# url-kaist/Quatro

Measured on NVIDIA H100. Metric: registrations/sec (64-ring pair), higher is better.
Workload: dtype f32 (front end, match, graph filter) / f64 (graph boundary, GNC, COTE)

## Files before the change

quatro_b200/csrc/api.cu:

```cuda
#include <cmath>
#include <new>
#include <stddef.h>
#include <stdio.h>
#include <stdlib.h>
#include <string.h>
#include <algorithm>
#include <map>
#include <mutex>
#include <utility>
#include <vector>

#include "handle.cuh"

using namespace qb;

namespace {

__global__ void wave_init_kernel(int* ctr_block, int n_ints, int* bbox, int n_clouds) {
  const int i = blockIdx.x * blockDim.x + threadIdx.x;
  if (i < n_ints) ctr_block[i] = 0;
  if (i < n_clouds * 6) bbox[i] = (i % 6) < 3 ? INT_MAX : INT_MIN;
}

__global__ void cache_copy_kernel(int to_cache, const int* __restrict__ slot_of_cloud, int V, float4* __restrict__ w_vox, float4* __restrict__ w_nrm,
// ... 75 lines not shown
  QB_CUDA_TRY(L, L->val_a.alloc(n_sort > n_hist ? n_sort : n_hist));
  QB_CUDA_TRY(L, L->val_b.alloc(n_sort));
  QB_CUDA_TRY(L, L->aos_scratch.alloc(2 * V * kDescDim));
  L->cub_bytes = sort_temp_bytes((int)(C * V));
  QB_CUDA_TRY(L, L->cub_temp.alloc_bytes(L->cub_bytes));
  QB_CUDA_TRY(L, L->vox_start.alloc(C * (V + 1)));
  QB_CUDA_TRY(L, L->vox_pts.alloc(C * V));
  QB_CUDA_TRY(L, L->cell_key.alloc(C * V));
  QB_CUDA_TRY(L, L->cell_start.alloc(C * (V + 1)));
  QB_CUDA_TRY(L, L->normals.alloc(C * V));
  QB_CUDA_TRY(L, L->spfh.alloc(C * V * kDescPad));
  QB_CUDA_TRY(L, L->nbr_list.alloc(C * kNbrGlobalCap * V));
  QB_CUDA_TRY(L, L->nbr_cnt.alloc(C * V));
  QB_CUDA_TRY(L, L->desc_t.alloc(C * kDescK * V));
  QB_CUDA_TRY(L, cudaMemset(L->desc_t, 0, C * kDescK * V * sizeof(float)));
  QB_CUDA_TRY(L, L->desc_tiles.alloc(C * kDescK * V * 3));
  QB_CUDA_TRY(L, cudaMemset(L->desc_tiles, 0, C * kDescK * V * 3 * sizeof(float)));
  QB_CUDA_TRY(L, L->desc_norm.alloc(C * V));
  QB_CUDA_TRY(L, L->tc_fallback.alloc(S));
  QB_CUDA_TRY(L, L->tc_stats.alloc(32));
  QB_CUDA_TRY(L, cudaMemset(L->tc_stats, 0, 32 * sizeof(unsigned long long)));
  QB_CUDA_TRY(L, L->rowbest.alloc(S * V));
  QB_CUDA_TRY(L, L->colpart.alloc(L->colpart_count()));
  QB_CUDA_TRY(L, L->colbest.alloc(S * V));
  QB_CUDA_TRY(L, L->mut_i.alloc(S * V));
  QB_CUDA_TRY(L, L->mut_j.alloc(S * V));
  QB_CUDA_TRY(L, L->mark.alloc(S * V));
  QB_CUDA_TRY(L, L->partner.alloc(S * V));
  QB_CUDA_TRY(L, L->mean.alloc(C * 4));
  QB_CUDA_TRY(L, L->corr_src.alloc(S * Lc));
  QB_CUDA_TRY(L, L->corr_tgt.alloc(S * Lc));
  QB_CUDA_TRY(L, L->ma.alloc(S * Lc));
// ... 1199 lines not shown
```

quatro_b200/csrc/common.cuh:

```cuda
#pragma once
#include <cuda_runtime.h>
#include <stdint.h>
#include <stdio.h>

#include "quatro_b200.h"

namespace qb {

constexpr int kOffIJ = 1 << 17;
constexpr int kOffK = 1 << 15;
constexpr uint64_t kCellMask = (1ull << 52) - 1;
constexpr uint64_t kCellInvalid = kCellMask;
constexpr int kCloudShift = 52;

__host__ __device__ __forceinline__ bool cell_ok(int i, int j, int k) {
  return i >= -kOffIJ && i < kOffIJ - 1 && j >= -kOffIJ && j < kOffIJ - 1 && k >= -kOffK && k < kOffK - 1;
}
__host__ __device__ __forceinline__ uint64_t cell_key(int i, int j, int k) {
  return ((uint64_t)(k + kOffK) << 36) | ((uint64_t)(j + kOffIJ) << 18) | (uint64_t)(i + kOffIJ);
}

constexpr int kVoxShift = 31;
constexpr uint64_t kVoxMask = (1ull << kVoxShift) - 1;
constexpr uint64_t kVoxInvalid = kVoxMask;
constexpr int kVsChunks = 64;
constexpr int kVsTile = 2048;

__device__ __forceinline__ bool raw_point_kept(const float4 p, int skip_flagged) {
  return isfinite(p.x) && isfinite(p.y) && isfinite(p.z) && !(skip_flagged && p.w < 0.0f);
}
__host__ __device__ __forceinline__ int vox_chunk_size(int n) { return n > 0 ? (n + kVsChunks - 1) / kVsChunks : 1; }

constexpr int kDescDim = 33;
constexpr int kDescPad = 36;
constexpr int kDescK = 40;
constexpr int kMatchTile = 128;
constexpr int kNbrGlobalCap = 80;

struct WaveCounters {
  int* n_valid;
  int* n_vox;
  int* n_lat;
  int* n_cells;
  int* cloud_status;
  int* bbox;
  int* vox_digits;
  int* n_mutual;
  int* n_corr;
  int* swapped;
  int* n_clique;
// ... 99 lines not shown
```

quatro_b200/csrc/tc_match.cu:

```cuda
#include "handle.cuh"
#include <cstdlib>

namespace qb {

constexpr int kTcM = 128, kTcN = 64;
constexpr int kTcBlk = 64;
constexpr int kTcKB = kDescK / 8;
constexpr int kTcTileBytes = kDescK * kTcBlk * 4;
constexpr int kTileFloats = kDescK * kTcBlk;
constexpr int kTcImages = 3;
constexpr int kTcEpiWarps = 8;
constexpr int kTcThreads = (kTcEpiWarps + 2) * 32;
constexpr int kTcDone = 4;
constexpr int kTcStages = 2;
constexpr int kTcSmemTiles = 256;
constexpr float kTcC = 1.2e-4f;
constexpr float kTcNormMax = 0x1p124f;
constexpr float kTcNormRel = 4.0e-6f;
constexpr int kSpinLimit = 400000;

__device__ __forceinline__ uint32_t smem_u32(const void* p) { return (uint32_t)__cvta_generic_to_shared(p); }

__device__ __forceinline__ uint64_t tc_smem_desc(uint32_t addr) {
  return (uint64_t)((addr & 0x3FFFF) >> 4) | ((uint64_t)((kTcBlk * 16) >> 4) << 16) | ((uint64_t)(128 >> 4) << 32);
}

__device__ __forceinline__ void wgmma_tf32_64x64x8(float (&d)[32], uint64_t adesc, uint64_t bdesc, int accumulate) {
  asm volatile(
      "{\n\t"
      ".reg .pred p;\n\t"
      "setp.ne.b32 p, %34, 0;\n\t"
      "wgmma.mma_async.sync.aligned.m64n64k8.f32.tf32.tf32 "
      "{%0, %1, %2, %3, %4, %5, %6, %7, %8, %9, %10, %11, %12, %13, %14, %15, "
      "%16, %17, %18, %19, %20, %21, %22, %23, %24, %25, %26, %27, %28, %29, %30, %31}, %32, %33, p, 1, 1;\n\t"
      "}\n"
      : "+f"(d[0]), "+f"(d[1]), "+f"(d[2]), "+f"(d[3]), "+f"(d[4]), "+f"(d[5]), "+f"(d[6]), "+f"(d[7]), "+f"(d[8]), "+f"(d[9]),
        "+f"(d[10]), "+f"(d[11]), "+f"(d[12]), "+f"(d[13]), "+f"(d[14]), "+f"(d[15]), "+f"(d[16]), "+f"(d[17]), "+f"(d[18]),
        "+f"(d[19]), "+f"(d[20]), "+f"(d[21]), "+f"(d[22]), "+f"(d[23]), "+f"(d[24]), "+f"(d[25]), "+f"(d[26]), "+f"(d[27]),
        "+f"(d[28]), "+f"(d[29]), "+f"(d[30]), "+f"(d[31])
      : "l"(adesc), "l"(bdesc), "r"(accumulate)
      : "memory");
}

__device__ __forceinline__ bool wg_all(bool v, int g) {
  uint32_t r;
  asm volatile(
      "{\n\t.reg .pred p, q;\n\t"
      "setp.ne.u32 p, %1, 0;\n\t"
      "bar.red.and.pred q, %2, 128, p;\n\t"
// ... 14 lines not shown
  uint32_t bits = 0xFFFFFFFFu;
  if (q < n_vox[cloud]) {
    const size_t base = (size_t)cloud * kDescK * V + q;
    float acc = 0.0f;
#pragma unroll
    for (int d = 0; d < kDescDim; ++d) {
      const float xc = desc_t[base + (size_t)d * V] - tc_mu(d);
      acc = __fmaf_rn(xc, xc, acc);
    }
    bits = acc == acc ? __float_as_uint(acc) : 0xFFFFFFFEu;
  }
  keys[(size_t)cloud * V + q] = ((uint64_t)cloud << 32) | bits;
  vals[(size_t)cloud * V + q] = (uint32_t)q;
}

__global__ void __launch_bounds__(256) split_desc_kernel(const float* __restrict__ desc_t, const int* __restrict__ n_vox, int V,
                                                         const uint32_t* __restrict__ perm, float* __restrict__ tiles,
                                                         float* __restrict__ norm, int* __restrict__ fallback) {
  const int cloud = blockIdx.y;
  const int q = blockIdx.x * blockDim.x + threadIdx.x;
  const int n = n_vox[cloud];
  const int NB = V / kTcBlk;
  if (q >= ((n + kTcM - 1) & ~(kTcM - 1))) return;
  const size_t base = (size_t)cloud * kDescK * V + (q < n ? perm[(size_t)cloud * V + q] : 0u);
  const int blk = q / kTcBlk, p = q % kTcBlk;
  float4* __restrict__ img = reinterpret_cast<float4*>(tiles + (size_t)(cloud * NB + blk) * kTcImages * kTileFloats) + p;
  const bool is_col = (cloud & 1) != 0;
  const float kLow = 1.0f - 0.5f * kTcC;
  float acc = 0.0f;
#pragma unroll
  for (int kc = 0; kc < kDescK / 4; ++kc) {
    float xv[4], hv[4], lv[4];
#pragma unroll
    for (int e = 0; e < 4; ++e) {
      const int d = 4 * kc + e;
      const bool live = d < kDescDim && q < n;
      const float x = live ? desc_t[base + (size_t)d * V] : 0.0f;
      const float xc = live ? x - tc_mu(d) : 0.0f;
      xv[e] = x;
      acc = __fmaf_rn(xc, xc, acc);
      float xs = is_col ? -2.0f * xc : xc;
      if (q < n && d == kDescDim) xs = is_col ? 1.0f : kLow * acc;
      if (q < n && d == kDescDim + 1) xs = is_col ? kLow * acc : 1.0f;
      hv[e] = __uint_as_float(__float_as_uint(xs) & 0xFFFFE000u);
      lv[e] = __uint_as_float(__float_as_uint(xs - hv[e]) & 0xFFFFE000u);
    }
    img[0 * (kTileFloats / 4) + kc * kTcBlk] = make_float4(hv[0], hv[1], hv[2], hv[3]);
    img[1 * (kTileFloats / 4) + kc * kTcBlk] = make_float4(lv[0], lv[1], lv[2], lv[3]);
    if (kc < kDescK / 4 - 1) img[2 * (kTileFloats / 4) + kc * kTcBlk] = make_float4(xv[0], xv[1], xv[2], xv[3]);
  }
  img[2 * (kTileFloats / 4) + (kDescK / 4 - 1) * kTcBlk] = make_float4(q < n ? kLow * acc : INFINITY, 0.0f, 0.0f, 0.0f);
  if (q < n) norm[(size_t)cloud * V + q] = acc;
  if (q < n && !(acc <= kTcNormMax)) fallback[cloud >> 1] = 1;
}

__global__ void __launch_bounds__(1024) dedup_kernel(const float* __restrict__ desc_t, const int* __restrict__ n_vox, int V,
                                                     const uint64_t* __restrict__ sorted_keys, const uint32_t* __restrict__ perm, int enable,
                                                     uint32_t* __restrict__ uperm, uint32_t* __restrict__ class_of, int* __restrict__ n_unique) {
  __shared__ int scan_smem[33];
  const int cloud = blockIdx.x;
  const int n = n_vox[cloud];
  const float* __restrict__ D = desc_t + (size_t)cloud * kDescK * V;
  const uint32_t* __restrict__ pm = perm + (size_t)cloud * V;
  const uint64_t* __restrict__ sk = sorted_keys + (size_t)cloud * V;
  int base = 0;
  for (int start = 0; start < n; start += blockDim.x) {
// ... 77 lines not shown
}
__device__ __forceinline__ unsigned tc_fkey(float f) {
  unsigned key = __float_as_uint(f);
  key = (key & 0x80000000u) ? ~key : (key | 0x80000000u);
  return f == f ? key : 0xFFFFFFFFu;
}
__device__ __forceinline__ float tc_fkey_inv(unsigned key) { return __uint_as_float((key & 0x80000000u) ? (key & 0x7FFFFFFFu) : ~key); }

template <bool kDbg, bool kProf = false>
__global__ void __launch_bounds__(kTcThreads, 2)
tc_nn_kernel(const float* __restrict__ tiles, const float* __restrict__ norm, const int* __restrict__ n_vox, int V,
             const uint32_t* __restrict__ perm, unsigned long long* __restrict__ rowbest, unsigned long long* __restrict__ colbest_r,
             unsigned* __restrict__ tile_cmax, int* __restrict__ fallback, unsigned long long* __restrict__ stats,
             float* __restrict__ dbg_tile) {
  extern __shared__ __align__(128) unsigned char smem[];
  __shared__ uint64_t s_fullx[kTcStages], s_sfree[kTcStages], s_fullhl, s_mma[kTcDone], s_afull;
  __shared__ unsigned long long s_rbest[kTcM];
  __shared__ __align__(16) float s_wcj[kTcEpiWarps][kTcN];
  __shared__ unsigned short s_queue[kTcEpiWarps][32];
  __shared__ int s_seq[8];
  __shared__ float s_tlb[kTcSmemTiles];
  __shared__ int s_dead, s_abort, s_evals, s_warm, s_npos;
  __shared__ int s_ndec;

  const int pair = blockIdx.y, stripe = blockIdx.x;
  const int cloudA = 2 * pair, cloudB = 2 * pair + 1;
  const int nA = n_vox[cloudA], nB = n_vox[cloudB];
  const int r0 = stripe * kTcM;
  if (r0 >= nA || nB <= 0) return;

  const int warp = threadIdx.x >> 5, lane = threadIdx.x & 31;
  const int NB = V / kTcBlk;
  auto tick = [&]() -> long long { return kProf ? clock64() : 0ll; };
  auto prof = [&](int slot, long long cyc) { if (kProf && lane == 0) atomicAdd(stats + slot, (unsigned long long)cyc); };
  const long long t_begin = tick();
  constexpr uint32_t kABytes = (kTcM / kTcBlk) * kTcImages * kTcTileBytes;
  constexpr uint32_t kHLBytes = 2 * kTcTileBytes;
  constexpr uint32_t kXBytes = kTcTileBytes;
  const uint32_t sA = smem_u32(smem), sHL = sA + kABytes, sX0 = sHL + kHLBytes;
  const float* __restrict__ tA = tiles + (size_t)cloudA * NB * kTcImages * kTileFloats;
  const float* __restrict__ tB = tiles + (size_t)cloudB * NB * kTcImages * kTileFloats;
  const float* __restrict__ nrmA = norm + (size_t)cloudA * V;
  const float* __restrict__ nrmB = norm + (size_t)cloudB * V;
  const uint32_t* __restrict__ permA = perm + (size_t)cloudA * V;
  const uint32_t* __restrict__ permB = perm + (size_t)cloudB * V;
  unsigned long long* __restrict__ cbg = colbest_r + (size_t)pair * V;
  const uint32_t bar_fullx0 = smem_u32(&s_fullx[0]), bar_sfree0 = smem_u32(&s_sfree[0]), bar_fullhl = smem_u32(&s_fullhl),
                 bar_mma0 = smem_u32(&s_mma[0]), bar_a = smem_u32(&s_afull);
  const int n_tiles = (nB + kTcN - 1) / kTcN;

  if (threadIdx.x == 0) {
    for (int i = 0; i < kTcStages; ++i) { mbar_init(bar_fullx0 + 8 * i, 1); mbar_init(bar_sfree0 + 8 * i, kTcEpiWarps); }
    mbar_init(bar_fullhl, 1);
    for (int i = 0; i < kTcDone; ++i) mbar_init(bar_mma0 + 8 * i, kTcEpiWarps);
    mbar_init(bar_a, 1);
    s_dead = 0; s_abort = 0; s_evals = 0; s_warm = 0; s_npos = 0; s_ndec = 0;
    asm volatile("fence.mbarrier_init.release.cluster;\n" ::: "memory");
  }
  if (threadIdx.x < kTcM) s_rbest[threadIdx.x] = ~0ull;
  __syncthreads();
  const long long t_setup = tick();
  if (kProf && threadIdx.x == 0) { atomicAdd(stats + 8, 1ull); atomicAdd(stats + 10, (unsigned long long)(t_setup - t_begin)); }
  volatile int* v_dead = &s_dead;
  volatile int* v_abort = &s_abort;
  volatile int* v_seq = s_seq;
  volatile int* v_ndec = &s_ndec;
  auto wait_decided = [&](int n) -> bool {
    for (int spin = 0; spin < kSpinLimit; ++spin) {
      if (*v_ndec > n) { __threadfence_block(); return true; }
      __nanosleep(32);
    }
    return false;
  };
  volatile unsigned long long* v_rbest = s_rbest;

  if (warp == kTcEpiWarps) {
    auto issue_hl = [&](int n) {
      const int t = v_seq[n & 7];
      if (lane != 0) return;
      if (t < 0) { mbar_arrive(bar_fullhl); return; }
      mbar_expect_tx(bar_fullhl, kHLBytes);
      bulk_g2s(sHL, tB + (size_t)t * kTcImages * kTileFloats, kHLBytes, bar_fullhl);
    };
    if (lane == 0) {
      mbar_expect_tx(bar_a, kABytes);
      bulk_g2s(sA, tA + (size_t)stripe * (kTcM / kTcBlk) * kTcImages * kTileFloats, kABytes, bar_a);
    }
    bool ok = wait_decided(0);
    if (ok) issue_hl(0);
    long long p_wm = 0, p_wd = 0;
    bool ended = !ok || v_seq[0] < 0;
    for (int k = 0; ok && !ended; ++k) {
      const long long t0 = tick();
      ok = mbar_wait(bar_mma0 + 8 * (k & (kTcDone - 1)), (uint32_t)((k >> 2) & 1));
      const long long t1 = tick();
      p_wm += t1 - t0;
      if (ok) ok = wait_decided(k + 1);
      p_wd += tick() - t1;
      if (!ok) break;
      issue_hl(k + 1);
      ended = v_seq[(k + 1) & 7] < 0;
    }
    prof(12, p_wm); prof(28, p_wd);
    if (!ok) *v_dead = 1;
  } else if (warp == kTcEpiWarps + 1) {
    const float amin = sqrtf(nrmA[r0]), amax = sqrtf(nrmA[(r0 + kTcM < nA ? r0 + kTcM : nA) - 1]);
    auto tile_lb = [&](int t) -> float {
      const float bmin = sqrtf(nrmB[t * kTcN]), bmax = sqrtf(nrmB[(t * kTcN + kTcN < nB ? t * kTcN + kTcN : nB) - 1]);
      const float gap = fmaxf(amin - bmax, bmin - amax) - (2.0e-3f + kTcNormRel * (amax + bmax));
      if (!(amin <= amax && bmin <= bmax)) return 0.0f;
      return gap > 0.0f ? gap * gap * 0.9999f : 0.0f;
    };
    constexpr int kPq = kTcSmemTiles / 32;
    const uint2* __restrict__ tcm2 = reinterpret_cast<const uint2*>(tile_cmax) + (size_t)pair * (V / kTcN);
    uint2 pq[kPq];
    auto fetch_tcm = [&]() {
// ... 73 lines not shown
      if (lane == 0) {
        v_seq[n & 7] = t;
        __threadfence_block();
        *v_ndec = n + 1;
      }
      __syncwarp();
      if (!done) fetch_tcm();
      return t;
    };
    auto issue_x = [&](int n) {
      const int t = v_seq[n & 7];
      if (lane != 0) return;
      const uint32_t bar = bar_fullx0 + 8 * (n % kTcStages);
      if (t < 0) { mbar_arrive(bar); return; }
      mbar_expect_tx(bar, kXBytes);
      bulk_g2s(sX0 + (n % kTcStages) * kXBytes, tB + ((size_t)t * kTcImages + 2) * kTileFloats, kXBytes, bar);
    };
    for (int n = 0; n < 3; ++n) {
      decide(n);
      if (n < kTcStages) issue_x(n);
    }
    prof(11, tick() - t_setup);
    long long p_wm = 0, p_dec = 0, p_sf = 0;
    auto mbar_test = [&](uint32_t bar, uint32_t parity) -> bool {
      uint32_t ready;
      asm volatile(
          "{\n\t.reg .pred p;\n\t"
          "mbarrier.test_wait.parity.shared::cta.b64 p, [%1], %2;\n\t"
          "selp.u32 %0, 1, 0, p;\n\t}\n"
          : "=r"(ready)
          : "r"(bar), "r"(parity)
// ... 23 lines not shown
        ++nd;
        p_dec += tick() - t1;
        continue;
      }
      if (idle == 0) t_idle = tick();
      if (++idle > kSpinLimit) { ok = false; break; }
      __nanosleep(32);
    }
    prof(29, p_wm); prof(13, p_dec); prof(14, p_sf);
    if (!ok) *v_dead = 1;
    if (lane == 0) s_npos = n_issued;
  } else {
    const int wg = warp >> 2;
    const int rbase = wg * 64 + 16 * (warp & 3);
    const int cl = 2 * (lane & 3);
    const float kLow = 1.0f - 0.5f * kTcC;
    const float kW = kTcC / kLow;
    bool row_ok[2];
    float nam[2], Ri_ub[2];
    unsigned oa[2];
#pragma unroll
    for (int h = 0; h < 2; ++h) {
      const int gi = r0 + rbase + (lane >> 2) + 8 * h;
      row_ok[h] = gi < nA;
      nam[h] = row_ok[h] ? kLow * nrmA[gi] : INFINITY;
      oa[h] = row_ok[h] ? permA[gi] : 0u;
      Ri_ub[h] = row_ok[h] ? INFINITY : -INFINITY;
    }
    const uint32_t row_bits = (row_ok[0] ? 0x33333333u : 0u) | (row_ok[1] ? 0xCCCCCCCCu : 0u);
    const float4* __restrict__ aex = reinterpret_cast<const float4*>(smem + (wg * kTcImages + 2) * kTcTileBytes);
    const uint32_t aH = sA + (uint32_t)(wg * kTcImages * kTcTileBytes), aL = aH + kTcTileBytes;
    float* wcj = s_wcj[warp];
    unsigned short* wq = s_queue[warp];
    int evals_w = 0;
    bool alive = mbar_wait(bar_a, 0);
    const long long t_loop = tick();
    prof(19, t_loop - t_setup);
    long long p_wx = 0, p_wmm = 0, p_ld = 0, p_prep = 0, p_fil = 0, p_ev = 0;
    int p_tiles = 0;
    int pf_tile = -1;
    unsigned long long pf_cb[2] = {~0ull, ~0ull};
    unsigned pf_ob[2] = {0u, 0u};
    unsigned* __restrict__ tcmw = tile_cmax + ((size_t)pair * (V / kTcN)) * 2;
    int rr_tile = -1;
    unsigned rr_val[2] = {0u, 0u};
    auto rr_flush = [&]() {
      if (rr_tile < 0) return;
#pragma unroll
      for (int s = 0; s < 2; ++s) {
        const unsigned m = __reduce_max_sync(0xffffffffu, rr_val[s]);
        if (lane == 0) atomicMin(tcmw + (size_t)rr_tile * 2 + s, m);
      }
      rr_tile = -1;
// ... 26 lines not shown
          const int jn = v_seq[(k + 1) & 7];
          if (jn >= 0) {
            pf_tile = jn;
#pragma unroll
            for (int s = 0; s < 2; ++s) {
              pf_cb[s] = ~0ull; pf_ob[s] = 0u;
              if (jn * kTcN + 32 * s + lane < nB) {
                pf_cb[s] = __ldcg(cbg + jn * kTcN + 32 * s + lane);
                pf_ob[s] = permB[jn * kTcN + 32 * s + lane];
              }
            }
          }
        }
      }
      const long long q2 = tick();
      if (alive && jt >= 0) alive = mbar_wait(bar_fullhl, (uint32_t)(k & 1));
      alive = __all_sync(0xffffffffu, alive);
      if (!wg_all(alive && jt >= 0, wg)) {
        if (!alive) *v_dead = 1;
        break;
      }
      float d[32];
#pragma unroll
      for (int i = 0; i < 32; ++i) d[i] = 0.0f;
      {
        constexpr uint32_t kKB = 2 * kTcBlk * 16;
        const uint32_t bH = sHL, bL = bH + kTcTileBytes;
        asm volatile("wgmma.fence.sync.aligned;\n" ::: "memory");
#pragma unroll
        for (int kb = 0; kb < kTcKB; ++kb) {
          wgmma_tf32_64x64x8(d, tc_smem_desc(aH + kb * kKB), tc_smem_desc(bL + kb * kKB), kb > 0);
          wgmma_tf32_64x64x8(d, tc_smem_desc(aL + kb * kKB), tc_smem_desc(bH + kb * kKB), 1);
        }
#pragma unroll
        for (int kb = 0; kb < kTcKB; ++kb) wgmma_tf32_64x64x8(d, tc_smem_desc(aH + kb * kKB), tc_smem_desc(bH + kb * kKB), 1);
        asm volatile("wgmma.commit_group.sync.aligned;\n" ::: "memory");
        asm volatile("wgmma.wait_group.sync.aligned 0;\n" ::: "memory");
#pragma unroll
        for (int i = 0; i < 32; ++i) asm volatile("" : "+f"(d[i])::"memory");
      }
      __syncwarp();
      if (lane == 0) mbar_arrive(bar_mma0 + 8 * ts);
      const long long q3 = tick();
      p_wmm += q3 - q2;
      p_prep += q2 - q1;
      ++p_tiles;
      const bool skip = __any_sync(0xffffffffu, (*v_abort | *v_dead) != 0);
      const long long q4 = tick();
      p_ld += q4 - q3;
      if (!skip) {
        const float4* __restrict__ bex = reinterpret_cast<const float4*>(smem + kABytes + kHLBytes + st * kXBytes);
        float dbest[2];
        bool col_warm = false;
#pragma unroll
        for (int s = 0; s < 2; ++s) {
          const float nbm = bex[9 * kTcBlk + 32 * s + lane].x;
          dbest[s] = cb_cur[s] == ~0ull ? INFINITY : __uint_as_float((unsigned)(cb_cur[s] >> 32));
          wcj[32 * s + lane] = nbm == INFINITY ? -INFINITY : dbest[s];
          col_warm |= cb_cur[s] == ~0ull && nbm != INFINITY;
        }
        float Ri[2];
        bool row_warm = false;
#pragma unroll
        for (int h = 0; h < 2; ++h) {
          const unsigned long long rb = v_rbest[rbase + (lane >> 2) + 8 * h];
          Ri[h] = fminf(Ri_ub[h], rb == ~0ull ? INFINITY : __uint_as_float((unsigned)(rb >> 32)));
          row_warm |= row_ok[h] && Ri[h] == INFINITY;
        }
        __syncwarp();
        if (__any_sync(0xffffffffu, row_warm || col_warm)) {
          if (lane == 0) atomicAdd(&s_warm, 1);
          float rowub[2] = {INFINITY, INFINITY};
#pragma unroll
          for (int i = 0; i < 32; i += 4) {
#pragma unroll
            for (int e = 0; e < 2; ++e) {
              const int c = 2 * i + cl + e;
              const float nbc = bex[9 * kTcBlk + c].x;
              const float ub0 = fmaf(kW, nam[0] + nbc, d[i + e]), ub1 = fmaf(kW, nam[1] + nbc, d[i + 2 + e]);
              rowub[0] = fminf(rowub[0], ub0);
              rowub[1] = fminf(rowub[1], ub1);
              unsigned mn = min(ub0 >= 0.0f ? __float_as_uint(ub0) : 0xFFFFFFFFu, ub1 >= 0.0f ? __float_as_uint(ub1) : 0xFFFFFFFFu);
              mn = min(mn, __shfl_xor_sync(0xffffffffu, mn, 4));
              mn = min(mn, __shfl_xor_sync(0xffffffffu, mn, 8));
              mn = min(mn, __shfl_xor_sync(0xffffffffu, mn, 16));
              if (lane < 4 && mn != 0xFFFFFFFFu && nbc != INFINITY) wcj[c] = fminf(wcj[c], __uint_as_float(mn));
            }
          }
#pragma unroll
          for (int h = 0; h < 2; ++h) {
            rowub[h] = fminf(rowub[h], __shfl_xor_sync(0xffffffffu, rowub[h], 1));
            rowub[h] = fminf(rowub[h], __shfl_xor_sync(0xffffffffu, rowub[h], 2));
            if (row_ok[h]) { Ri_ub[h] = fminf(Ri_ub[h], rowub[h]); Ri[h] = fminf(Ri[h], Ri_ub[h]); }
          }
        }
        __syncwarp();
        const long long q5 = tick();
        p_prep += q5 - q4;
        const int ncol = nB - c0;
        uint32_t mask = 0, col_bits = 0;
#pragma unroll
// ... 1 lines not shown
          const float2 x = *reinterpret_cast<const float2*>(wcj + 2 * i + cl);
#pragma unroll
          for (int e = 0; e < 4; ++e) {
            const float lbv = d[i + e];
            const float xc = (e & 1) ? x.y : x.x;
            asm("{\n\t.reg .pred p, q;\n\t"
                "setp.le.f32 p, %1, %2;\n\t"
                "setp.le.or.f32 q, %1, %3, p;\n\t"
                "@q or.b32 %0, %0, %4;\n\t}\n"
                : "+r"(mask)
                : "f"(lbv), "f"(xc), "f"(Ri[e >> 1]), "r"(1u << (i + e)));
            if (2 * i + cl + (e & 1) < ncol) col_bits |= 1u << (i + e);
            if (kDbg) {
              const int h = e >> 1, c = 2 * i + cl + (e & 1);
              if (stripe == 0 && row_ok[h] && c < ncol)
                dbg_tile[(size_t)oa[h] * 128 + permB[c0 + c]] = fmaf(0.5f * kW, nam[h] + bex[9 * kTcBlk + c].x, lbv);
            }
          }
        }
        mask &= col_bits & row_bits;
        int remaining = __reduce_add_sync(0xffffffffu, __popc(mask));
        const long long q6 = tick();
        p_fil += q6 - q5;
        evals_w += remaining;
        while (remaining > 0) {
          int tot;
          int p = warp_excl_scan(__popc(mask), &tot);
          while (mask && p < 32) {
            const int i = __ffs(mask) - 1;
            mask &= mask - 1;
            wq[p++] = (unsigned short)((lane << 5) | i);
// ... 39 lines not shown
      if (lane == 0) mbar_arrive(bar_sfree0 + 8 * st);
      rr_flush();
      if (!skip) {
        rr_tile = jt;
#pragma unroll
        for (int s = 0; s < 2; ++s) {
          rr_val[s] = 0;
          if (c0 + 32 * s + lane < nB) {
            const unsigned long long cbn = __ldcg(cbg + c0 + 32 * s + lane);
            rr_val[s] = cbn == ~0ull ? 0x7F800000u : (unsigned)(cbn >> 32);
          }
        }
      }
    }
    rr_flush();
    prof(20, p_wx); prof(21, p_wmm); prof(22, p_ld); prof(23, p_prep); prof(24, p_fil); prof(25, p_ev);
    prof(26, tick() - t_loop); prof(27, p_tiles);
  }
  __syncthreads();
  const bool aborted = (s_abort | s_dead) != 0;
  if (kProf && threadIdx.x == 0) atomicAdd(stats + 9, (unsigned long long)(tick() - t_begin));
  if (threadIdx.x == 0) {
    atomicAdd(stats + 0, (unsigned long long)s_evals);
    atomicAdd(stats + 1, (unsigned long long)s_npos);
    atomicAdd(stats + 2, (unsigned long long)s_warm);
    if (aborted) {
      atomicAdd(stats + 3, 1ull);
      fallback[pair] = 1;
    }
  }
  if (!aborted && threadIdx.x < kTcM && r0 + (int)threadIdx.x < nA) rowbest[(size_t)pair * V + r0 + threadIdx.x] = s_rbest[threadIdx.x];
}

static size_t tc_smem_bytes() {
  return ((size_t)(kTcM / kTcBlk) * kTcImages + 2 + kTcStages) * kTcTileBytes;
}

static int tc_prepare(Lane* h, const void* kernel) {
  QB_CUDA_TRY(h, ensure_dyn_smem(h->device, kernel, tc_smem_bytes()));
  QB_CUDA_TRY(h, cudaFuncSetAttribute(kernel, cudaFuncAttributePreferredSharedMemoryCarveout, cudaSharedmemCarveoutMaxShared));
  return QB200_OK;
}

int tc_footprint(Lane* h, int* out5) {
  const void* kernel = (const void*)tc_nn_kernel<false>;
  if (int rc = tc_prepare(h, kernel)) return rc;
  cudaFuncAttributes fa;
  QB_CUDA_TRY(h, cudaFuncGetAttributes(&fa, kernel));
  int ctas = 0;
  QB_CUDA_TRY(h, cudaOccupancyMaxActiveBlocksPerMultiprocessor(&ctas, kernel, kTcThreads, tc_smem_bytes()));
  out5[0] = kTcThreads;
// ... 25 lines not shown
  const size_t smem = tc_smem_bytes();
  if (int rc = tc_prepare(h, (const void*)tc_nn_kernel<false>)) return rc;
  int rc = sort_and_dedup(h, 2 * n_pairs, 1);
  if (rc) return rc;
  const uint32_t* uperm = h->val_a;
  const uint32_t* class_of = h->class_of();
  const int* n_unique = h->n_unique();
  unsigned long long* colbest_u = h->colpart_col();
  unsigned long long* rowbest_u = h->colpart_row();
  unsigned* tile_cmax = h->colpart_tile_cmax();
  QB_CUDA_TRY(h, cudaMemsetAsync(h->rowbest, 0xFF, (size_t)n_pairs * V * 8, h->stream));
  QB_CUDA_TRY(h, cudaMemsetAsync(h->colbest, 0xFF, (size_t)n_pairs * V * 8, h->stream));
  QB_CUDA_TRY(h, cudaMemsetAsync(h->colpart, 0xFF, h->colpart_count() * 8, h->stream));
  QB_CUDA_TRY(h, cudaMemsetAsync(h->tc_fallback, 0, (size_t)n_pairs * sizeof(int), h->stream));
  const dim3 gsplit((V + 255) / 256, 2 * n_pairs);
  split_desc_kernel<<<gsplit, 256, 0, h->stream>>>(h->desc_t, n_unique, V, uperm, h->desc_tiles, h->desc_norm, h->tc_fallback);
  const dim3 g(h->NS, n_pairs);
  cudaEventRecord(h->kev[0], h->stream);
  if (h->tc_prof) {
    if (int rc2 = tc_prepare(h, (const void*)tc_nn_kernel<false, true>)) return rc2;
    tc_nn_kernel<false, true><<<g, kTcThreads, smem, h->stream>>>(h->desc_tiles, h->desc_norm, n_unique, V, uperm, rowbest_u, colbest_u,
                                                                  tile_cmax, h->tc_fallback, h->tc_stats, nullptr);
  } else {
    tc_nn_kernel<false><<<g, kTcThreads, smem, h->stream>>>(h->desc_tiles, h->desc_norm, n_unique, V, uperm, rowbest_u, colbest_u,
                                                            tile_cmax, h->tc_fallback, h->tc_stats, nullptr);
  }
  cudaEventRecord(h->kev[1], h->stream);
  h->kev_armed[0] = 1;
  broadcast_best_kernel<<<gsplit, 256, 0, h->stream>>>(rowbest_u, colbest_u, h->ctr.n_vox, V, h->val_b, class_of, h->rowbest, h->colbest);
  h->launches += 3;
  QB_CUDA_TRY(h, cudaGetLastError());
  return launch_match_exact(h, n_pairs, h->tc_fallback);
}

int launch_tc_debug_tile(Lane* h, float* d_out) {
  const size_t smem = tc_smem_bytes();
  if (int rc0 = tc_prepare(h, (const void*)tc_nn_kernel<true>)) return rc0;
  int rc = sort_and_dedup(h, 2, 0);
  if (rc) return rc;
  const uint32_t* uperm = h->val_a;
  const int* n_unique = h->n_unique();
  QB_CUDA_TRY(h, cudaMemsetAsync(h->colpart, 0xFF, h->colpart_count() * 8, h->stream));
  QB_CUDA_TRY(h, cudaMemsetAsync(h->tc_fallback, 0, sizeof(int), h->stream));
  const dim3 gsplit((h->V + 255) / 256, 2);
  split_desc_kernel<<<gsplit, 256, 0, h->stream>>>(h->desc_t, n_unique, h->V, uperm, h->desc_tiles, h->desc_norm, h->tc_fallback);
  const dim3 g(1, 1);
  tc_nn_kernel<true><<<g, kTcThreads, smem, h->stream>>>(h->desc_tiles, h->desc_norm, n_unique, h->V, uperm, h->colpart_row(), h->colpart_col(),
                                                         h->colpart_tile_cmax(), h->tc_fallback, h->tc_stats, d_out);
  h->launches += 2;
  QB_CUDA_TRY(h, cudaGetLastError());
  return QB200_OK;
}

}
```

Before: 13590.

## Switch descriptor NN matching from split-TF32 to split-FP16 WGMMA with pair scaling

Replaces the hi/lo TF32 split with FP16 hi/lo operand images packed at K=48, which halves operand bytes and uses m64n64k16 f16 WGMMA instead of k8 tf32. A per-pair power-of-two scale keeps values in half range, and an error bound term computed in the split kernel goes into the extra image so the epilogue's upper-bound filter stays conservative. It also double-buffers the B hi/lo operand loads and adds a third stage for the exact-value tiles. The cost is more complex error accounting that must stay conservative for correctness, and a fixed 100 KB shared-memory footprint.

```diff
diff --git a/quatro_b200/csrc/api.cu b/quatro_b200/csrc/api.cu
--- a/quatro_b200/csrc/api.cu
+++ b/quatro_b200/csrc/api.cu
@@ -113,8 +113,8 @@
   QB_CUDA_TRY(L, L->nbr_cnt.alloc(C * V));
   QB_CUDA_TRY(L, L->desc_t.alloc(C * kDescK * V));
   QB_CUDA_TRY(L, cudaMemset(L->desc_t, 0, C * kDescK * V * sizeof(float)));
-  QB_CUDA_TRY(L, L->desc_tiles.alloc(C * kDescK * V * 3));
-  QB_CUDA_TRY(L, cudaMemset(L->desc_tiles, 0, C * kDescK * V * 3 * sizeof(float)));
+  QB_CUDA_TRY(L, L->desc_tiles.alloc(C * (V / 64) * kTcBlockFloats));
+  QB_CUDA_TRY(L, cudaMemset(L->desc_tiles, 0, C * (V / 64) * kTcBlockFloats * sizeof(float)));
   QB_CUDA_TRY(L, L->desc_norm.alloc(C * V));
   QB_CUDA_TRY(L, L->tc_fallback.alloc(S));
   QB_CUDA_TRY(L, L->tc_stats.alloc(32));
diff --git a/quatro_b200/csrc/common.cuh b/quatro_b200/csrc/common.cuh
--- a/quatro_b200/csrc/common.cuh
+++ b/quatro_b200/csrc/common.cuh
@@ -34,6 +34,8 @@
 constexpr int kDescDim = 33;
 constexpr int kDescPad = 36;
 constexpr int kDescK = 40;
+constexpr int kTcOpK = 48;
+constexpr int kTcBlockFloats = (2 * 64 * kTcOpK * 2 + 64 * kDescK * 4) / 4;
 constexpr int kMatchTile = 128;
 constexpr int kNbrGlobalCap = 80;
 
diff --git a/quatro_b200/csrc/tc_match.cu b/quatro_b200/csrc/tc_match.cu
--- a/quatro_b200/csrc/tc_match.cu
+++ b/quatro_b200/csrc/tc_match.cu
@@ -1,18 +1,22 @@
 #include "handle.cuh"
+#include <cuda_fp16.h>
 #include <cstdlib>
 
 namespace qb {
 
 constexpr int kTcM = 128, kTcN = 64;
 constexpr int kTcBlk = 64;
-constexpr int kTcKB = kDescK / 8;
-constexpr int kTcTileBytes = kDescK * kTcBlk * 4;
-constexpr int kTileFloats = kDescK * kTcBlk;
-constexpr int kTcImages = 3;
+constexpr int kTcKS = kTcOpK / 16;
+constexpr int kTcOpBytes = kTcOpK * kTcBlk * 2;
+constexpr int kTcExBytes = kDescK * kTcBlk * 4;
+static_assert(2 * kTcOpBytes + kTcExBytes == kTcBlockFloats * 4, "operand-image block layout (common.cuh)");
+constexpr int kTcBlkBytes = kTcBlockFloats * 4;
 constexpr int kTcEpiWarps = 8;
 constexpr int kTcThreads = (kTcEpiWarps + 2) * 32;
 constexpr int kTcDone = 4;
-constexpr int kTcStages = 2;
+constexpr int kTcOpStages = 2;
+constexpr int kTcStages = 3;
+constexpr int kTcDynSmem = 100 * 1024;
 constexpr int kTcSmemTiles = 256;
 constexpr float kTcC = 1.2e-4f;
 constexpr float kTcNormMax = 0x1p124f;
@@ -25,14 +29,14 @@
   return (uint64_t)((addr & 0x3FFFF) >> 4) | ((uint64_t)((kTcBlk * 16) >> 4) << 16) | ((uint64_t)(128 >> 4) << 32);
 }
 
-__device__ __forceinline__ void wgmma_tf32_64x64x8(float (&d)[32], uint64_t adesc, uint64_t bdesc, int accumulate) {
+__device__ __forceinline__ void wgmma_f16_64x64x16(float (&d)[32], uint64_t adesc, uint64_t bdesc, int accumulate) {
   asm volatile(
       "{\n\t"
       ".reg .pred p;\n\t"
       "setp.ne.b32 p, %34, 0;\n\t"
-      "wgmma.mma_async.sync.aligned.m64n64k8.f32.tf32.tf32 "
+      "wgmma.mma_async.sync.aligned.m64n64k16.f32.f16.f16 "
       "{%0, %1, %2, %3, %4, %5, %6, %7, %8, %9, %10, %11, %12, %13, %14, %15, "
-      "%16, %17, %18, %19, %20, %21, %22, %23, %24, %25, %26, %27, %28, %29, %30, %31}, %32, %33, p, 1, 1;\n\t"
+      "%16, %17, %18, %19, %20, %21, %22, %23, %24, %25, %26, %27, %28, %29, %30, %31}, %32, %33, p, 1, 1, 0, 0;\n\t"
       "}\n"
       : "+f"(d[0]), "+f"(d[1]), "+f"(d[2]), "+f"(d[3]), "+f"(d[4]), "+f"(d[5]), "+f"(d[6]), "+f"(d[7]), "+f"(d[8]), "+f"(d[9]),
         "+f"(d[10]), "+f"(d[11]), "+f"(d[12]), "+f"(d[13]), "+f"(d[14]), "+f"(d[15]), "+f"(d[16]), "+f"(d[17]), "+f"(d[18]),
@@ -77,8 +81,17 @@
   vals[(size_t)cloud * V + q] = (uint32_t)q;
 }
 
+__device__ __forceinline__ float tc_pair_scale(float ma, float mb) {
+  const float m = fmaxf(ma, mb);
+  if (!(ma <= kTcNormMax && mb <= kTcNormMax && m > 0.0f)) return 1.0f;
+  const int e = (ilogbf(m) - 13) >> 1;
+  return __int_as_float((127 - e) << 23);
+}
+__device__ __forceinline__ float tc_scaled_up(float thr, float s) { return __fmul_ru(__fmul_ru(thr, s), s); }
+
 __global__ void __launch_bounds__(256) split_desc_kernel(const float* __restrict__ desc_t, const int* __restrict__ n_vox, int V,
-                                                         const uint32_t* __restrict__ perm, float* __restrict__ tiles,
+                                                         const uint32_t* __restrict__ perm, const uint64_t* __restrict__ sorted_keys,
+                                                         const int* __restrict__ n_all, float* __restrict__ tiles,
                                                          float* __restrict__ norm, int* __restrict__ fallback) {
   const int cloud = blockIdx.y;
   const int q = blockIdx.x * blockDim.x + threadIdx.x;
@@ -87,32 +100,61 @@
   if (q >= ((n + kTcM - 1) & ~(kTcM - 1))) return;
   const size_t base = (size_t)cloud * kDescK * V + (q < n ? perm[(size_t)cloud * V + q] : 0u);
   const int blk = q / kTcBlk, p = q % kTcBlk;
-  float4* __restrict__ img = reinterpret_cast<float4*>(tiles + (size_t)(cloud * NB + blk) * kTcImages * kTileFloats) + p;
+  unsigned char* __restrict__ blkp = reinterpret_cast<unsigned char*>(tiles) + (size_t)(cloud * NB + blk) * kTcBlkBytes + p * 16;
+  uint4* __restrict__ hi_img = reinterpret_cast<uint4*>(blkp);
+  uint4* __restrict__ lo_img = reinterpret_cast<uint4*>(blkp + kTcOpBytes);
+  float4* __restrict__ ex_img = reinterpret_cast<float4*>(blkp + 2 * kTcOpBytes);
+  auto max_norm = [&](int c) {
+    const int m = n_all[c];
+    return m > 0 ? __uint_as_float((uint32_t)sorted_keys[(size_t)c * V + m - 1]) : 0.0f;
+  };
+  const float s = tc_pair_scale(max_norm(cloud & ~1), max_norm(cloud | 1));
   const bool is_col = (cloud & 1) != 0;
   const float kLow = 1.0f - 0.5f * kTcC;
-  float acc = 0.0f;
-#pragma unroll
-  for (int kc = 0; kc < kDescK / 4; ++kc) {
-    float xv[4], hv[4], lv[4];
-#pragma unroll
-    for (int e = 0; e < 4; ++e) {
-      const int d = 4 * kc + e;
+  const float kW = kTcC / kLow;
+  float acc = 0.0f, l1 = 0.0f, ub_term = INFINITY, nres = 0.0f;
+#pragma unroll
+  for (int kc = 0; kc < kTcOpK / 8; ++kc) {
+    float xv[8];
+    __half hv[8], lv[8];
+#pragma unroll
+    for (int e = 0; e < 8; ++e) {
+      const int d = 8 * kc + e;
       const bool live = d < kDescDim && q < n;
       const float x = live ? desc_t[base + (size_t)d * V] : 0.0f;
       const float xc = live ? x - tc_mu(d) : 0.0f;
       xv[e] = x;
       acc = __fmaf_rn(xc, xc, acc);
-      float xs = is_col ? -2.0f * xc : xc;
-      if (q < n && d == kDescDim) xs = is_col ? 1.0f : kLow * acc;
-      if (q < n && d == kDescDim + 1) xs = is_col ? kLow * acc : 1.0f;
-      hv[e] = __uint_as_float(__float_as_uint(xs) & 0xFFFFE000u);
-      lv[e] = __uint_as_float(__float_as_uint(xs - hv[e]) & 0xFFFFE000u);
-    }
-    img[0 * (kTileFloats / 4) + kc * kTcBlk] = make_float4(hv[0], hv[1], hv[2], hv[3]);
-    img[1 * (kTileFloats / 4) + kc * kTcBlk] = make_float4(lv[0], lv[1], lv[2], lv[3]);
-    if (kc < kDescK / 4 - 1) img[2 * (kTileFloats / 4) + kc * kTcBlk] = make_float4(xv[0], xv[1], xv[2], xv[3]);
+      float xs = (is_col ? -2.0f * xc : xc) * s;
+      l1 += fabsf(xs);
+      const int j = d - kDescDim;
+      const bool own = (j & 1) == (int)is_col;
+      if (q < n && j >= 0 && j < 4) {
+        if (j == 0) {
+          const float nt = kLow * acc * s * s;
+          const float eps = __fmaf_ru(0x1p-23f, l1, 0x1p-40f);
+          ub_term = __fmaf_ru(kW, nt, 2.0f * eps);
+          nres = __fsub_rd(nt, eps);
+        }
+        xs = j < 2 ? (own ? nres : 1.0f) : (own ? nres * 0x1p20f : 0x1p-20f);
+      }
+      hv[e] = __float2half_rn(xs);
+      lv[e] = __float2half_rn(xs - __half2float(hv[e]));
+      if (q < n && j >= 0 && j < 2 && own) nres = (xs - __half2float(hv[e])) - __half2float(lv[e]);
+    }
+    auto pack = [](const __half (&h)[8]) {
+      uint32_t w[4];
+#pragma unroll
+      for (int j = 0; j < 4; ++j) w[j] = (uint32_t)__half_as_ushort(h[2 * j]) | ((uint32_t)__half_as_ushort(h[2 * j + 1]) << 16);
+      return make_uint4(w[0], w[1], w[2], w[3]);
+    };
+    hi_img[kc * kTcBlk] = pack(hv);
+    lo_img[kc * kTcBlk] = pack(lv);
+#pragma unroll
+    for (int j = 0; j < 2; ++j)
+      if (2 * kc + j < kDescK / 4 - 1) ex_img[(2 * kc + j) * kTcBlk] = make_float4(xv[4 * j], xv[4 * j + 1], xv[4 * j + 2], xv[4 * j + 3]);
   }
-  img[2 * (kTileFloats / 4) + (kDescK / 4 - 1) * kTcBlk] = make_float4(q < n ? kLow * acc : INFINITY, 0.0f, 0.0f, 0.0f);
+  ex_img[(kDescK / 4 - 1) * kTcBlk] = make_float4(q < n ? kLow * acc : INFINITY, ub_term, 0.0f, 0.0f);
   if (q < n) norm[(size_t)cloud * V + q] = acc;
   if (q < n && !(acc <= kTcNormMax)) fallback[cloud >> 1] = 1;
 }
@@ -220,7 +262,7 @@
              unsigned* __restrict__ tile_cmax, int* __restrict__ fallback, unsigned long long* __restrict__ stats,
              float* __restrict__ dbg_tile) {
   extern __shared__ __align__(128) unsigned char smem[];
-  __shared__ uint64_t s_fullx[kTcStages], s_sfree[kTcStages], s_fullhl, s_mma[kTcDone], s_afull;
+  __shared__ uint64_t s_fullx[kTcStages], s_sfree[kTcStages], s_fullhl[kTcOpStages], s_mma[kTcDone], s_afull;
   __shared__ unsigned long long s_rbest[kTcM];
   __shared__ __align__(16) float s_wcj[kTcEpiWarps][kTcN];
   __shared__ unsigned short s_queue[kTcEpiWarps][32];
@@ -240,24 +282,26 @@
   auto tick = [&]() -> long long { return kProf ? clock64() : 0ll; };
   auto prof = [&](int slot, long long cyc) { if (kProf && lane == 0) atomicAdd(stats + slot, (unsigned long long)cyc); };
   const long long t_begin = tick();
-  constexpr uint32_t kABytes = (kTcM / kTcBlk) * kTcImages * kTcTileBytes;
-  constexpr uint32_t kHLBytes = 2 * kTcTileBytes;
-  constexpr uint32_t kXBytes = kTcTileBytes;
-  const uint32_t sA = smem_u32(smem), sHL = sA + kABytes, sX0 = sHL + kHLBytes;
-  const float* __restrict__ tA = tiles + (size_t)cloudA * NB * kTcImages * kTileFloats;
-  const float* __restrict__ tB = tiles + (size_t)cloudB * NB * kTcImages * kTileFloats;
+  constexpr uint32_t kABytes = (kTcM / kTcBlk) * kTcBlkBytes;
+  constexpr uint32_t kHLBytes = 2 * kTcOpBytes;
+  constexpr uint32_t kXBytes = kTcExBytes;
+  constexpr uint32_t kXOff = kABytes + kTcOpStages * kHLBytes;
+  static_assert(kXOff + kTcStages * kXBytes <= kTcDynSmem, "shared-memory map");
+  const uint32_t sA = smem_u32(smem), sHL = sA + kABytes, sX0 = sA + kXOff;
+  const unsigned char* __restrict__ tA = reinterpret_cast<const unsigned char*>(tiles) + (size_t)cloudA * NB * kTcBlkBytes;
+  const unsigned char* __restrict__ tB = reinterpret_cast<const unsigned char*>(tiles) + (size_t)cloudB * NB * kTcBlkBytes;
   const float* __restrict__ nrmA = norm + (size_t)cloudA * V;
   const float* __restrict__ nrmB = norm + (size_t)cloudB * V;
   const uint32_t* __restrict__ permA = perm + (size_t)cloudA * V;
   const uint32_t* __restrict__ permB = perm + (size_t)cloudB * V;
   unsigned long long* __restrict__ cbg = colbest_r + (size_t)pair * V;
-  const uint32_t bar_fullx0 = smem_u32(&s_fullx[0]), bar_sfree0 = smem_u32(&s_sfree[0]), bar_fullhl = smem_u32(&s_fullhl),
+  const uint32_t bar_fullx0 = smem_u32(&s_fullx[0]), bar_sfree0 = smem_u32(&s_sfree[0]), bar_fullhl0 = smem_u32(&s_fullhl[0]),
                  bar_mma0 = smem_u32(&s_mma[0]), bar_a = smem_u32(&s_afull);
   const int n_tiles = (nB + kTcN - 1) / kTcN;
 
   if (threadIdx.x == 0) {
     for (int i = 0; i < kTcStages; ++i) { mbar_init(bar_fullx0 + 8 * i, 1); mbar_init(bar_sfree0 + 8 * i, kTcEpiWarps); }
-    mbar_init(bar_fullhl, 1);
+    for (int i = 0; i < kTcOpStages; ++i) mbar_init(bar_fullhl0 + 8 * i, 1);
     for (int i = 0; i < kTcDone; ++i) mbar_init(bar_mma0 + 8 * i, kTcEpiWarps);
     mbar_init(bar_a, 1);
     s_dead = 0; s_abort = 0; s_evals = 0; s_warm = 0; s_npos = 0; s_ndec = 0;
@@ -284,28 +328,31 @@
     auto issue_hl = [&](int n) {
       const int t = v_seq[n & 7];
       if (lane != 0) return;
-      if (t < 0) { mbar_arrive(bar_fullhl); return; }
-      mbar_expect_tx(bar_fullhl, kHLBytes);
-      bulk_g2s(sHL, tB + (size_t)t * kTcImages * kTileFloats, kHLBytes, bar_fullhl);
+      const uint32_t bar = bar_fullhl0 + 8 * (n % kTcOpStages);
+      if (t < 0) { mbar_arrive(bar); return; }
+      mbar_expect_tx(bar, kHLBytes);
+      bulk_g2s(sHL + (n % kTcOpStages) * kHLBytes, tB + (size_t)t * kTcBlkBytes, kHLBytes, bar);
     };
     if (lane == 0) {
       mbar_expect_tx(bar_a, kABytes);
-      bulk_g2s(sA, tA + (size_t)stripe * (kTcM / kTcBlk) * kTcImages * kTileFloats, kABytes, bar_a);
-    }
-    bool ok = wait_decided(0);
-    if (ok) issue_hl(0);
+      bulk_g2s(sA, tA + (size_t)stripe * (kTcM / kTcBlk) * kTcBlkBytes, kABytes, bar_a);
+    }
+    bool ok = true, ended = false;
+    for (int n = 0; n < kTcOpStages && ok && !ended; ++n) {
+      ok = wait_decided(n);
+      if (ok) { issue_hl(n); ended = v_seq[n & 7] < 0; }
+    }
     long long p_wm = 0, p_wd = 0;
-    bool ended = !ok || v_seq[0] < 0;
     for (int k = 0; ok && !ended; ++k) {
       const long long t0 = tick();
       ok = mbar_wait(bar_mma0 + 8 * (k & (kTcDone - 1)), (uint32_t)((k >> 2) & 1));
       const long long t1 = tick();
       p_wm += t1 - t0;
-      if (ok) ok = wait_decided(k + 1);
+      if (ok) ok = wait_decided(k + kTcOpStages);
       p_wd += tick() - t1;
       if (!ok) break;
-      issue_hl(k + 1);
-      ended = v_seq[(k + 1) & 7] < 0;
+      issue_hl(k + kTcOpStages);
+      ended = v_seq[(k + kTcOpStages) & 7] < 0;
     }
     prof(12, p_wm); prof(28, p_wd);
     if (!ok) *v_dead = 1;
@@ -409,7 +456,7 @@
       const uint32_t bar = bar_fullx0 + 8 * (n % kTcStages);
       if (t < 0) { mbar_arrive(bar); return; }
       mbar_expect_tx(bar, kXBytes);
-      bulk_g2s(sX0 + (n % kTcStages) * kXBytes, tB + ((size_t)t * kTcImages + 2) * kTileFloats, kXBytes, bar);
+      bulk_g2s(sX0 + (n % kTcStages) * kXBytes, tB + (size_t)t * kTcBlkBytes + 2 * kTcOpBytes, kXBytes, bar);
     };
     for (int n = 0; n < 3; ++n) {
       decide(n);
@@ -463,29 +510,29 @@
     const int wg = warp >> 2;
     const int rbase = wg * 64 + 16 * (warp & 3);
     const int cl = 2 * (lane & 3);
-    const float kLow = 1.0f - 0.5f * kTcC;
-    const float kW = kTcC / kLow;
+    const float sc = tc_pair_scale(nrmA[nA - 1], nrmB[nB - 1]);
     bool row_ok[2];
-    float nam[2], Ri_ub[2];
+    float ta[2], Ri_ub[2];
     unsigned oa[2];
 #pragma unroll
     for (int h = 0; h < 2; ++h) {
       const int gi = r0 + rbase + (lane >> 2) + 8 * h;
       row_ok[h] = gi < nA;
-      nam[h] = row_ok[h] ? kLow * nrmA[gi] : INFINITY;
       oa[h] = row_ok[h] ? permA[gi] : 0u;
       Ri_ub[h] = row_ok[h] ? INFINITY : -INFINITY;
     }
     const uint32_t row_bits = (row_ok[0] ? 0x33333333u : 0u) | (row_ok[1] ? 0xCCCCCCCCu : 0u);
-    const float4* __restrict__ aex = reinterpret_cast<const float4*>(smem + (wg * kTcImages + 2) * kTcTileBytes);
-    const uint32_t aH = sA + (uint32_t)(wg * kTcImages * kTcTileBytes), aL = aH + kTcTileBytes;
+    const float4* __restrict__ aex = reinterpret_cast<const float4*>(smem + wg * kTcBlkBytes + 2 * kTcOpBytes);
+    const uint32_t aH = sA + (uint32_t)(wg * kTcBlkBytes), aL = aH + kTcOpBytes;
     float* wcj = s_wcj[warp];
     unsigned short* wq = s_queue[warp];
     int evals_w = 0;
     bool alive = mbar_wait(bar_a, 0);
+#pragma unroll
+    for (int h = 0; h < 2; ++h) ta[h] = aex[9 * kTcBlk + 16 * (warp & 3) + (lane >> 2) + 8 * h].y;
     const long long t_loop = tick();
     prof(19, t_loop - t_setup);
-    long long p_wx = 0, p_wmm = 0, p_ld = 0, p_prep = 0, p_fil = 0, p_ev = 0;
+    long long p_wx = 0, p_whl = 0, p_wmm = 0, p_ld = 0, p_prep = 0, p_fil = 0, p_ev = 0;
     int p_tiles = 0;
     int pf_tile = -1;
     unsigned long long pf_cb[2] = {~0ull, ~0ull};
@@ -542,26 +589,27 @@
         }
       }
       const long long q2 = tick();
-      if (alive && jt >= 0) alive = mbar_wait(bar_fullhl, (uint32_t)(k & 1));
+      if (alive && jt >= 0) alive = mbar_wait(bar_fullhl0 + 8 * (k % kTcOpStages), (uint32_t)((k / kTcOpStages) & 1));
       alive = __all_sync(0xffffffffu, alive);
       if (!wg_all(alive && jt >= 0, wg)) {
         if (!alive) *v_dead = 1;
         break;
       }
+      const long long q2m = tick();
       float d[32];
 #pragma unroll
       for (int i = 0; i < 32; ++i) d[i] = 0.0f;
       {
-        constexpr uint32_t kKB = 2 * kTcBlk * 16;
-        const uint32_t bH = sHL, bL = bH + kTcTileBytes;
+        constexpr uint32_t kKS = 2 * kTcBlk * 16;
+        const uint32_t bH = sHL + (k % kTcOpStages) * kHLBytes, bL = bH + kTcOpBytes;
         asm volatile("wgmma.fence.sync.aligned;\n" ::: "memory");
 #pragma unroll
-        for (int kb = 0; kb < kTcKB; ++kb) {
-          wgmma_tf32_64x64x8(d, tc_smem_desc(aH + kb * kKB), tc_smem_desc(bL + kb * kKB), kb > 0);
-          wgmma_tf32_64x64x8(d, tc_smem_desc(aL + kb * kKB), tc_smem_desc(bH + kb * kKB), 1);
-        }
-#pragma unroll
-        for (int kb = 0; kb < kTcKB; ++kb) wgmma_tf32_64x64x8(d, tc_smem_desc(aH + kb * kKB), tc_smem_desc(bH + kb * kKB), 1);
+        for (int ks = 0; ks < kTcKS; ++ks) {
+          wgmma_f16_64x64x16(d, tc_smem_desc(aH + ks * kKS), tc_smem_desc(bL + ks * kKS), ks > 0);
+          wgmma_f16_64x64x16(d, tc_smem_desc(aL + ks * kKS), tc_smem_desc(bH + ks * kKS), 1);
+        }
+#pragma unroll
+        for (int ks = 0; ks < kTcKS; ++ks) wgmma_f16_64x64x16(d, tc_smem_desc(aH + ks * kKS), tc_smem_desc(bH + ks * kKS), 1);
         asm volatile("wgmma.commit_group.sync.aligned;\n" ::: "memory");
         asm volatile("wgmma.wait_group.sync.aligned 0;\n" ::: "memory");
 #pragma unroll
@@ -570,21 +618,22 @@
       __syncwarp();
       if (lane == 0) mbar_arrive(bar_mma0 + 8 * ts);
       const long long q3 = tick();
-      p_wmm += q3 - q2;
+      p_whl += q2m - q2;
+      p_wmm += q3 - q2m;
       p_prep += q2 - q1;
       ++p_tiles;
       const bool skip = __any_sync(0xffffffffu, (*v_abort | *v_dead) != 0);
       const long long q4 = tick();
       p_ld += q4 - q3;
       if (!skip) {
-        const float4* __restrict__ bex = reinterpret_cast<const float4*>(smem + kABytes + kHLBytes + st * kXBytes);
+        const float4* __restrict__ bex = reinterpret_cast<const float4*>(smem + kXOff + st * kXBytes);
         float dbest[2];
         bool col_warm = false;
 #pragma unroll
         for (int s = 0; s < 2; ++s) {
           const float nbm = bex[9 * kTcBlk + 32 * s + lane].x;
           dbest[s] = cb_cur[s] == ~0ull ? INFINITY : __uint_as_float((unsigned)(cb_cur[s] >> 32));
-          wcj[32 * s + lane] = nbm == INFINITY ? -INFINITY : dbest[s];
+          wcj[32 * s + lane] = nbm == INFINITY ? -INFINITY : tc_scaled_up(dbest[s], sc);
           col_warm |= cb_cur[s] == ~0ull && nbm != INFINITY;
         }
         float Ri[2];
@@ -592,7 +641,7 @@
 #pragma unroll
         for (int h = 0; h < 2; ++h) {
           const unsigned long long rb = v_rbest[rbase + (lane >> 2) + 8 * h];
-          Ri[h] = fminf(Ri_ub[h], rb == ~0ull ? INFINITY : __uint_as_float((unsigned)(rb >> 32)));
+          Ri[h] = fminf(Ri_ub[h], rb == ~0ull ? INFINITY : tc_scaled_up(__uint_as_float((unsigned)(rb >> 32)), sc));
           row_warm |= row_ok[h] && Ri[h] == INFINITY;
         }
         __syncwarp();
@@ -604,15 +653,15 @@
 #pragma unroll
             for (int e = 0; e < 2; ++e) {
               const int c = 2 * i + cl + e;
-              const float nbc = bex[9 * kTcBlk + c].x;
-              const float ub0 = fmaf(kW, nam[0] + nbc, d[i + e]), ub1 = fmaf(kW, nam[1] + nbc, d[i + 2 + e]);
+              const float2 nbc = *reinterpret_cast<const float2*>(&bex[9 * kTcBlk + c]);
+              const float ub0 = d[i + e] + (ta[0] + nbc.y), ub1 = d[i + 2 + e] + (ta[1] + nbc.y);
               rowub[0] = fminf(rowub[0], ub0);
               rowub[1] = fminf(rowub[1], ub1);
               unsigned mn = min(ub0 >= 0.0f ? __float_as_uint(ub0) : 0xFFFFFFFFu, ub1 >= 0.0f ? __float_as_uint(ub1) : 0xFFFFFFFFu);
               mn = min(mn, __shfl_xor_sync(0xffffffffu, mn, 4));
               mn = min(mn, __shfl_xor_sync(0xffffffffu, mn, 8));
               mn = min(mn, __shfl_xor_sync(0xffffffffu, mn, 16));
-              if (lane < 4 && mn != 0xFFFFFFFFu && nbc != INFINITY) wcj[c] = fminf(wcj[c], __uint_as_float(mn));
+              if (lane < 4 && mn != 0xFFFFFFFFu && nbc.x != INFINITY) wcj[c] = fminf(wcj[c], __uint_as_float(mn));
             }
           }
 #pragma unroll
@@ -644,7 +693,7 @@
             if (kDbg) {
               const int h = e >> 1, c = 2 * i + cl + (e & 1);
               if (stripe == 0 && row_ok[h] && c < ncol)
-                dbg_tile[(size_t)oa[h] * 128 + permB[c0 + c]] = fmaf(0.5f * kW, nam[h] + bex[9 * kTcBlk + c].x, lbv);
+                dbg_tile[(size_t)oa[h] * 128 + permB[c0 + c]] = (lbv + 0.5f * (ta[h] + bex[9 * kTcBlk + c].y)) / sc / sc;
             }
           }
         }
@@ -714,7 +763,7 @@
       }
     }
     rr_flush();
-    prof(20, p_wx); prof(21, p_wmm); prof(22, p_ld); prof(23, p_prep); prof(24, p_fil); prof(25, p_ev);
+    prof(20, p_wx); prof(21, p_whl); prof(30, p_wmm); prof(22, p_ld); prof(23, p_prep); prof(24, p_fil); prof(25, p_ev);
     prof(26, tick() - t_loop); prof(27, p_tiles);
   }
   __syncthreads();
@@ -732,9 +781,7 @@
   if (!aborted && threadIdx.x < kTcM && r0 + (int)threadIdx.x < nA) rowbest[(size_t)pair * V + r0 + threadIdx.x] = s_rbest[threadIdx.x];
 }
 
-static size_t tc_smem_bytes() {
-  return ((size_t)(kTcM / kTcBlk) * kTcImages + 2 + kTcStages) * kTcTileBytes;
-}
+static size_t tc_smem_bytes() { return kTcDynSmem; }
 
 static int tc_prepare(Lane* h, const void* kernel) {
   QB_CUDA_TRY(h, ensure_dyn_smem(h->device, kernel, tc_smem_bytes()));
@@ -790,7 +837,8 @@
   QB_CUDA_TRY(h, cudaMemsetAsync(h->colpart, 0xFF, h->colpart_count() * 8, h->stream));
   QB_CUDA_TRY(h, cudaMemsetAsync(h->tc_fallback, 0, (size_t)n_pairs * sizeof(int), h->stream));
   const dim3 gsplit((V + 255) / 256, 2 * n_pairs);
-  split_desc_kernel<<<gsplit, 256, 0, h->stream>>>(h->desc_t, n_unique, V, uperm, h->desc_tiles, h->desc_norm, h->tc_fallback);
+  split_desc_kernel<<<gsplit, 256, 0, h->stream>>>(h->desc_t, n_unique, V, uperm, h->key_b, h->ctr.n_vox, h->desc_tiles, h->desc_norm,
+                                                   h->tc_fallback);
   const dim3 g(h->NS, n_pairs);
   cudaEventRecord(h->kev[0], h->stream);
   if (h->tc_prof) {
@@ -819,7 +867,8 @@
   QB_CUDA_TRY(h, cudaMemsetAsync(h->colpart, 0xFF, h->colpart_count() * 8, h->stream));
   QB_CUDA_TRY(h, cudaMemsetAsync(h->tc_fallback, 0, sizeof(int), h->stream));
   const dim3 gsplit((h->V + 255) / 256, 2);
-  split_desc_kernel<<<gsplit, 256, 0, h->stream>>>(h->desc_t, n_unique, h->V, uperm, h->desc_tiles, h->desc_norm, h->tc_fallback);
+  split_desc_kernel<<<gsplit, 256, 0, h->stream>>>(h->desc_t, n_unique, h->V, uperm, h->key_b, h->ctr.n_vox, h->desc_tiles, h->desc_norm,
+                                                   h->tc_fallback);
   const dim3 g(1, 1);
   tc_nn_kernel<true><<<g, kTcThreads, smem, h->stream>>>(h->desc_tiles, h->desc_norm, n_unique, h->V, uperm, h->colpart_row(), h->colpart_col(),
                                                          h->colpart_tile_cmax(), h->tc_fallback, h->tc_stats, d_out);
```

Result: faster. 13980, median of 6 (+2.9%).
